# TaceoLabs/co-snarks

Measured on NVIDIA H100. Metric: co-Groth16 proofs/sec (BN254, 2^20 constraints); MSM Mscalar/s, higher is better.
Workload: dtype u32x8 (256-bit Montgomery, integer)

## Files before the change

### co_snarks_b200/csrc/cs_api.cu

```cuda
#include <stdarg.h>
#include "cs_lib.cuh"

namespace cs {

std::string& last_error() {
  static thread_local std::string e;
  return e;
}
int fail(int code, const char* fmt, ...) {
  char buf[1024];
  va_list ap;
  va_start(ap, fmt);
  vsnprintf(buf, sizeof(buf), fmt, ap);
  va_end(ap);
  last_error() = buf;
  return code;
}
#if !defined(CS_EMU)
__attribute__((constructor)) static void cs_more_hw_queues() { setenv("CUDA_DEVICE_MAX_CONNECTIONS", "32", 0); }
#endif

std::atomic<uint64_t>& launch_counter() {
  static std::atomic<uint64_t> c{0};
  return c;
}

int ctx_fork(cs_ctx* ctx, int nside) {
  if (ctx->msm_ws[0].profile) {
    if (!ctx->ev_t0) CS_CUDA(cudaEventCreateWithFlags(&ctx->ev_t0, 0));
    CS_CUDA(cudaEventRecord(ctx->ev_t0, ctx->stream));
  }
  CS_CUDA(cudaEventRecord(ctx->ev_fork, ctx->stream));
  for (int i = 0; i < nside; i++) CS_CUDA(cudaStreamWaitEvent(ctx->side[i], ctx->ev_fork, 0));
  return 0;
}
int ctx_join(cs_ctx* ctx, int nside) {
  for (int i = 0; i < nside; i++) {
    CS_CUDA(cudaEventRecord(ctx->ev_side[i], ctx->side[i]));
    CS_CUDA(cudaStreamWaitEvent(ctx->stream, ctx->ev_side[i], 0));
  }
  return 0;
}

template <class FrP>
static int ntt_smem_optin() {
#if !defined(CS_EMU)
#define CS_NTT_ATTR(D, S, KB) \
  CS_CUDA(cudaFuncSetAttribute(k_ntt_pass<FrP, D, S>, cudaFuncAttributeMaxDynamicSharedMemorySize, KB * 1024))
  CS_NTT_ATTR(true, false, 64); CS_NTT_ATTR(false, false, 64); CS_NTT_ATTR(true, true, 96); CS_NTT_ATTR(false, true, 96);
#undef CS_NTT_ATTR
#endif
  return 0;
}

}

using namespace cs;

extern "C" {

const char* cs_last_error(void) { return last_error().c_str(); }

const char* cs_version(void) {
#if defined(CS_EMU)
  return "cosnarks-b200 0.1 (CPU emulation build -- tests only)";
#else
  return "cosnarks-b200 0.1 (sm_90a)";
#endif
}

int cs_ctx_create(int device, void* stream, cs_ctx** out) {
  if (!out) return fail(CS_ERR_ARG, "cs_ctx_create: out is NULL");
  int ndev = 0;
  cudaError_t e = cudaGetDeviceCount(&ndev);
  if (e != cudaSuccess || ndev == 0)
    return fail(CS_ERR_CUDA, "cs_ctx_create: no CUDA device available (%s); this library has no CPU path",
                e != cudaSuccess ? cudaGetErrorString(e) : "device count 0");
  if (device < 0 || device >= ndev) return fail(CS_ERR_ARG, "cs_ctx_create: device %d out of range (%d devices)", device, ndev);
  CS_CUDA(cudaSetDevice(device));
  cs_ctx* ctx = new cs_ctx();
  ctx->device = device;
  int prio_side = -2, prio_acc = 0, prio_wm = -2;
  if (const char* e = getenv("CS_PRIO")) sscanf(e, "%d,%d,%d", &prio_side, &prio_acc, &prio_wm);
  const char* split_env = getenv("CS_MSM_SPLIT");
  const bool split = !(split_env && atoi(split_env) == 0);
  if (stream) {
    ctx->stream = (cudaStream_t)stream;
  } else {
    CS_CUDA(cudaStreamCreateWithPriority(&ctx->stream, cudaStreamNonBlocking, prio_side));
    ctx->own_stream = true;
  }
  for (int i = 0; i < CS_NSIDE; i++) {
    CS_CUDA(cudaStreamCreateWithPriority(&ctx->side[i], cudaStreamNonBlocking, prio_side));
    if (split) CS_CUDA(cudaStreamCreateWithPriority(&ctx->acc[i], cudaStreamNonBlocking, prio_acc));
    CS_CUDA(cudaEventCreateWithFlags(&ctx->ev_side[i], cudaEventDisableTiming));
  }
  CS_CUDA(cudaStreamCreateWithPriority(&ctx->wm, cudaStreamNonBlocking, prio_wm));
  CS_CUDA(cudaEventCreateWithFlags(&ctx->ev_wm, cudaEventDisableTiming));
  CS_CUDA(cudaEventCreateWithFlags(&ctx->ev_fork, cudaEventDisableTiming));
  CS_TRY(ntt_smem_optin<Bn254Fr>());
#if defined(CS_ENABLE_BLS12_381)
  CS_TRY(ntt_smem_optin<Bls381Fr>());
#endif
  *out = ctx;
  return 0;
}

void cs_ctx_destroy(cs_ctx* ctx) {
  if (!ctx) return;
  cudaSetDevice(ctx->device);
  cudaDeviceSynchronize();
  ctx->msm_ws[CS_WIT_SORT].release();
  for (int i = 0; i < CS_NSIDE; i++) {
    ctx->msm_ws[i].release();
    if (ctx->side[i]) cudaStreamDestroy(ctx->side[i]);
    if (ctx->acc[i]) cudaStreamDestroy(ctx->acc[i]);
    if (ctx->ev_side[i]) cudaEventDestroy(ctx->ev_side[i]);
  }
  if (ctx->ev_fork) cudaEventDestroy(ctx->ev_fork);
  if (ctx->wm) cudaStreamDestroy(ctx->wm);
  if (ctx->ev_wm) cudaEventDestroy(ctx->ev_wm);
  if (ctx->ev_t0) cudaEventDestroy(ctx->ev_t0);
  ctx->io.release();
  ctx->prf_keys.release();
  ctx->sc_part.release();
  ctx->sc_res.release();
  if (ctx->own_stream && ctx->stream) cudaStreamDestroy(ctx->stream);
  delete ctx;
}

int cs_ctx_synchronize(cs_ctx* ctx) {
  if (!ctx) return fail(CS_ERR_ARG, "ctx is NULL");
  CS_CUDA(cudaStreamSynchronize(ctx->stream));
  return 0;
}

uint64_t cs_ctx_launch_count(const cs_ctx*) { return launch_counter().load(); }

int cs_dev_alloc(cs_ctx* ctx, size_t bytes, void** d_out) {
  if (!ctx || !d_out) return fail(CS_ERR_ARG, "cs_dev_alloc: bad argument");
  CS_CUDA(cudaSetDevice(ctx->device));
  CS_CUDA(cudaMalloc(d_out, bytes ? bytes : 1));
  return 0;
}
int cs_dev_free(cs_ctx* ctx, void* d_ptr) {
  if (!ctx) return fail(CS_ERR_ARG, "ctx is NULL");
  CS_CUDA(cudaFree(d_ptr));
  return 0;
}
int cs_host_alloc_pinned(size_t bytes, void** h_out) {
  if (!h_out) return fail(CS_ERR_ARG, "h_out is NULL");
  CS_CUDA(cudaMallocHost(h_out, bytes ? bytes : 1));
  return 0;
}
int cs_host_free_pinned(void* h_ptr) {
  CS_CUDA(cudaFreeHost(h_ptr));
  return 0;
}
int cs_memcpy_h2d(cs_ctx* ctx, void* d_dst, const void* h_src, size_t bytes) {
  if (!ctx) return fail(CS_ERR_ARG, "ctx is NULL");
  CS_CUDA(cudaMemcpyAsync(d_dst, h_src, bytes, cudaMemcpyHostToDevice, ctx->stream));
  CS_CUDA(cudaStreamSynchronize(ctx->stream));
  return 0;
}
int cs_memcpy_d2h(cs_ctx* ctx, void* h_dst, const void* d_src, size_t bytes) {
  if (!ctx) return fail(CS_ERR_ARG, "ctx is NULL");
  CS_CUDA(cudaMemcpyAsync(h_dst, d_src, bytes, cudaMemcpyDeviceToHost, ctx->stream));
  CS_CUDA(cudaStreamSynchronize(ctx->stream));
  return 0;
}

}

namespace cs {

constexpr unsigned MSM_MAX_WINDOW = 20;
static_assert((1u << (MSM_MAX_WINDOW - 1)) + 1 <= MSM_SCAN_MAX_BLOCKS * MSM_SCAN_T, "MSM_MAX_WINDOW exceeds the scan");

template <class Cfg, int G>
int bases_upload_t(cs_ctx* ctx, const uint64_t* h_points, size_t n, int window_bits, cs_bases* b) {
  typedef typename GroupOf<Cfg, G>::F F;
  unsigned c = window_bits ? (unsigned)window_bits : msm_auto_window(n, Cfg::FR_BITS);
  if (c < 2 || c > MSM_MAX_WINDOW)
    return fail(CS_ERR_ARG, "cs_bases_upload: window_bits %d out of range [2,%u] (0 = automatic)", window_bits, MSM_MAX_WINDOW);
  b->sh = msm_shape(Cfg::FR_BITS, c);
  b->n = n;
  size_t total = (size_t)b->sh.W * n;
  if (total >= (1ull << 31)) return fail(CS_ERR_LIMIT, "cs_bases_upload: W*n = %zu exceeds 2^31", total);
  CS_TRY(b->table.reserve(total * sizeof(Affine<F>)));
  CS_CUDA(cudaMemcpyAsync(b->table.p, h_points, n * sizeof(Affine<F>), cudaMemcpyHostToDevice, ctx->stream));
  CS_TRY(b->infmask.reserve(((n + 31) / 32) * 4));
  CS_LAUNCH(k_msm_infmask<F>, ceil_div((n + 31) / 32, 128), 128, 0, ctx->stream, b->table.as<Affine<F>>(), (uint32_t)n,
            b->infmask.as<uint32_t>());
  CS_LAUNCH(k_msm_precompute<F>, ceil_div(n, 128), 128, 0, ctx->stream, b->table.as<Affine<F>>(), (uint32_t)n,
            b->sh.c, b->sh.W);
  if (G == 0 && std::is_same<Cfg, Bn254Cfg>::value) {
    static int f52_env = -1;
    if (f52_env < 0) { const char* e = getenv("CS_MSM_F52"); f52_env = e ? atoi(e) : 0; }
    if (f52_env) {
      const size_t ncoords = total * 2;
      CS_LAUNCH(k_msm_table_to_m260<Bn254Fq52 COMMA Bn254Fq>, ceil_div(ncoords, 128), 128, 0, ctx->stream,
                b->table.as<uint32_t>(), ncoords);
      b->m260 = true;
    }
  }
  CS_CUDA(cudaGetLastError());
  CS_CUDA(cudaStreamSynchronize(ctx->stream));
  return 0;
}

template <class Cfg, int G>
int msm_enqueue_t(cs_ctx* ctx, int slot, cudaStream_t st, const cs_bases* b, size_t offset,
                  const uint32_t* d_scalars, unsigned sstride, size_t n, int mont, int sort_slot, bool view) {
  typedef typename GroupOf<Cfg, G>::F F;
  return msm_enqueue<F, typename Cfg::FrP>(ctx->msm_ws[slot], b->table.as<Affine<F>>(), b->infmask.as<uint32_t>(), (uint32_t)b->n, b->sh,
                                           (uint32_t)offset, d_scalars, sstride, (uint32_t)n, mont, st,
                                           sort_slot >= 0 ? &ctx->msm_ws[sort_slot] : nullptr, view, b->m260, ctx->acc[slot]);
}

template <class Cfg, int G>
void msm_finish_t(cs_ctx* ctx, int slot, uint64_t* out_affine, int* out_inf) {
  typedef typename GroupOf<Cfg, G>::HF HF;
  const host::HXyzz<HF>* r = reinterpret_cast<const host::HXyzz<HF>*>(ctx->msm_ws[slot].h_result);
  host::HAffine<HF> a = host::haffine(*r);
  memcpy(out_affine, &a, sizeof(a));
  if (out_inf) *out_inf = a.is_inf() ? 1 : 0;
}

int msm_enqueue_dyn(cs_ctx* ctx, int slot, cudaStream_t st, const cs_bases* b, size_t offset,
                    const uint32_t* d_scalars, unsigned sstride, size_t n, int mont, int sort_slot, bool view) {
  CS_DISPATCH_CURVE(b->curve, {
    if (b->group == CS_G1) return msm_enqueue_t<Cfg, 0>(ctx, slot, st, b, offset, d_scalars, sstride, n, mont, sort_slot, view);
    return msm_enqueue_t<Cfg, 1>(ctx, slot, st, b, offset, d_scalars, sstride, n, mont, sort_slot, view);
  });
  return 0;
}
int msm_sort_shared_dyn(cs_ctx* ctx, int slot, cudaStream_t st, const cs_bases* b, const uint32_t* d_scalars,
                        unsigned sstride, size_t n, int mont) {
  CS_DISPATCH_CURVE(b->curve, {
    return msm_sort<typename Cfg::FrP>(ctx->msm_ws[slot], nullptr, (uint32_t)n, b->sh, 0, d_scalars, sstride, (uint32_t)n,
                                       mont, st);
  });
  return 0;
}

int msm_finish_dyn(cs_ctx* ctx, int slot, const cs_bases* b, uint64_t* out_affine, int* out_inf) {
  CS_DISPATCH_CURVE(b->curve, {
    if (b->group == CS_G1) msm_finish_t<Cfg, 0>(ctx, slot, out_affine, out_inf);
    else msm_finish_t<Cfg, 1>(ctx, slot, out_affine, out_inf);
  });
  return 0;
}

}

// ... 834 lines not shown
```

### co_snarks_b200/csrc/cs_msm.cuh

```cuda
#pragma once
#include <stdlib.h>
#include "cs_common.cuh"
#include "cs_curve.cuh"

namespace cs {

constexpr unsigned MSM_SLICE_MAX = 64;
constexpr unsigned MSM_ORDER_BLOCK = 256;
constexpr unsigned MSM_RED_SEG = 4;
constexpr unsigned MSM_SIGN = 0x80000000u;

template <class FrP>
CS_GLOBAL void k_msm_digits(const uint32_t* __restrict__ scalars, uint32_t sstride, uint32_t n, int mont,
                            uint32_t c, uint32_t W, const uint32_t* __restrict__ infmask, uint32_t offset,
                            uint32_t* __restrict__ dig, uint32_t* __restrict__ count) {
  uint32_t i = blockIdx.x * blockDim.x + threadIdx.x;
  if (i >= n) return;
  if (infmask && ((infmask[(offset + i) >> 5] >> ((offset + i) & 31)) & 1)) {
    for (uint32_t w = 0; w < W; w++) dig[(size_t)w * n + i] = 0;
    return;
  }
  Fp<FrP> s;
  const uint4* src = reinterpret_cast<const uint4*>(scalars) + (size_t)i * sstride * (FrP::N / 4);
  CS_UNROLL
  for (int k = 0; k < FrP::N / 4; k++) {
    uint4 v = src[k];
    s.l[4 * k] = v.x; s.l[4 * k + 1] = v.y; s.l[4 * k + 2] = v.z; s.l[4 * k + 3] = v.w;
  }
  if (mont) s = s.from_mont();
  uint32_t lim[FrP::N + 1];
  CS_UNROLL
  for (int k = 0; k < FrP::N; k++) lim[k] = s.l[k];
  lim[FrP::N] = 0;
  const uint32_t half = 1u << (c - 1);
  const uint32_t mask = (1u << c) - 1;
  uint32_t carry = 0;
  for (uint32_t w = 0; w < W; w++) {
    uint32_t pos = w * c;
    uint32_t li = pos >> 5, sh = pos & 31;
    uint32_t lo = li < FrP::N ? lim[li] : 0;
    uint32_t hi = li + 1 < FrP::N ? lim[li + 1] : 0;
    uint32_t d = (__funnelshift_r(lo, hi, sh) & mask) + carry;
    uint32_t out;
    if (d > half) {
      out = ((1u << c) - d) | MSM_SIGN;
      carry = 1;
    } else {
      out = d;
      carry = 0;
    }
    dig[(size_t)w * n + i] = out;
    uint32_t b = out & ~MSM_SIGN;
    if (b) atomicAdd(&count[b], 1u);
  }
}

template <class F>
CS_GLOBAL void k_msm_infmask(const Affine<F>* __restrict__ table, uint32_t n, uint32_t* __restrict__ mask) {
  uint32_t wd = blockIdx.x * blockDim.x + threadIdx.x;
  if (wd * 32 >= n) return;
  uint32_t m = 0;
  for (uint32_t k = 0; k < 32 && wd * 32 + k < n; k++)
    if (table[wd * 32 + k].is_inf()) m |= 1u << k;
  mask[wd] = m;
}

constexpr unsigned MSM_SCAN_T = 1024;
constexpr unsigned MSM_SCAN_MAX_BLOCKS = 1024;
CS_D void msm_scan_terms(const uint32_t* __restrict__ count, uint32_t k, uint32_t nb1, uint32_t S, uint32_t* v) {
  uint32_t cnt = (k && k < nb1) ? count[k] : 0;
  uint32_t n0 = (cnt + S - 1) / S;
  uint32_t n1 = (n0 + S - 1) / S;
  v[0] = cnt; v[1] = n0; v[2] = n1; v[3] = (n1 + S - 1) / S;
}
static CS_GLOBAL void k_msm_scan1(const uint32_t* __restrict__ count, uint32_t nb1 , uint32_t S,
                                  uint32_t* __restrict__ start, uint32_t* __restrict__ sstart0,
                                  uint32_t* __restrict__ sstart1, uint32_t* __restrict__ sstart2, uint32_t* __restrict__ aux) {
  __shared__ uint32_t sm[4][32];
  const uint32_t t = threadIdx.x, lane = t & 31, wid = t >> 5, nwarp = blockDim.x >> 5;
  const uint32_t k = blockIdx.x * blockDim.x + t;
  uint32_t v[4], inc[4];
  msm_scan_terms(count, k, nb1, S, v);
  CS_UNROLL
  for (int q = 0; q < 4; q++) {
    uint32_t x = v[q];
    CS_UNROLL
    for (uint32_t d = 1; d < 32; d <<= 1) {
      uint32_t y = __shfl_up_sync(0xffffffffu, x, d);
      if (lane >= d) x += y;
    }
    inc[q] = x;
    if (lane == 31) sm[q][wid] = x;
  }
  __syncthreads();
  uint32_t w[4], x[4];
  CS_UNROLL
  for (int q = 0; q < 4; q++) {
    w[q] = (wid == 0 && lane < nwarp) ? sm[q][lane] : 0;
    x[q] = w[q];
    CS_UNROLL
    for (uint32_t d = 1; d < 32; d <<= 1) {
      uint32_t y = __shfl_up_sync(0xffffffffu, x[q], d);
      if (lane >= d) x[q] += y;
    }
  }
  __syncthreads();
  if (wid == 0 && lane < nwarp) {
    CS_UNROLL
    for (int q = 0; q < 4; q++) sm[q][lane] = x[q] - w[q];
    if (lane == nwarp - 1) {
      CS_UNROLL
      for (int q = 0; q < 4; q++) aux[blockIdx.x * 4 + q] = x[q];
    }
  }
  __syncthreads();
  if (k < nb1) {
    start[k] = sm[0][wid] + inc[0] - v[0];
    sstart0[k] = sm[1][wid] + inc[1] - v[1];
    sstart1[k] = sm[2][wid] + inc[2] - v[2];
    sstart2[k] = sm[3][wid] + inc[3] - v[3];
  }
}
static CS_GLOBAL void k_msm_scan2(const uint32_t* __restrict__ count, uint32_t nb1, uint32_t S,
                                  uint32_t* __restrict__ start, uint32_t* __restrict__ sstart0,
                                  uint32_t* __restrict__ sstart1, uint32_t* __restrict__ sstart2,
                                  const uint32_t* __restrict__ aux) {
  const uint32_t k = blockIdx.x * blockDim.x + threadIdx.x;
  if (k >= nb1) return;
  uint32_t off[4] = {0, 0, 0, 0};
  for (uint32_t b = 0; b < blockIdx.x; b++) {
    CS_UNROLL
    for (int q = 0; q < 4; q++) off[q] += aux[b * 4 + q];
  }
  uint32_t a = start[k] + off[0], b0 = sstart0[k] + off[1], b1 = sstart1[k] + off[2], b2 = sstart2[k] + off[3];
  start[k] = a; sstart0[k] = b0; sstart1[k] = b1; sstart2[k] = b2;
  if (k == nb1 - 1) {
    uint32_t v[4];
    msm_scan_terms(count, k, nb1, S, v);
    start[nb1] = a + v[0]; sstart0[nb1] = b0 + v[1]; sstart1[nb1] = b1 + v[2]; sstart2[nb1] = b2 + v[3];
  }
}

static CS_GLOBAL void k_msm_scatter(const uint32_t* __restrict__ dig, uint32_t n, uint32_t nbases,
                             uint32_t offset, const uint32_t* __restrict__ start,
                             uint32_t* __restrict__ cursor, uint32_t* __restrict__ sorted) {
  uint32_t i = blockIdx.x * blockDim.x + threadIdx.x;
  uint32_t w = blockIdx.y;
  if (i >= n) return;
  uint32_t d = dig[(size_t)w * n + i];
  uint32_t b = d & ~MSM_SIGN;
  if (!b) return;
  uint32_t pos = start[b] + atomicAdd(&cursor[b], 1u);
  sorted[pos] = (w * nbases + offset + i) | (d & MSM_SIGN);
}

constexpr unsigned MSM_VIEW_T = 256;
constexpr unsigned MSM_VIEW_WORDS = MSM_VIEW_T / 32;

CS_D uint32_t popc32(uint32_t x) {
#if defined(CS_EMU)
  return (uint32_t)__builtin_popcount(x);
#else
  return __popc(x);
#endif
}
CS_D uint32_t warp_bits(bool pred) {
#if defined(CS_EMU)
  uint32_t x = pred ? 1u << (threadIdx.x & 31) : 0u;
  for (uint32_t d = 16; d > 0; d >>= 1) x += __shfl_xor_sync(0xffffffffu, x, d);
  return x;
#else
  return __ballot_sync(0xffffffffu, pred);
#endif
}

static CS_GLOBAL void k_msm_view_flags(const uint32_t* __restrict__ sorted, const uint32_t* __restrict__ src_start,
                                       uint32_t nb1, uint32_t n, const uint32_t* __restrict__ infmask, uint32_t offset,
                                       uint32_t* __restrict__ keep, uint32_t* __restrict__ blk_cnt) {
  __shared__ uint32_t cnt[MSM_VIEW_WORDS];
  const uint32_t t = threadIdx.x;
  const uint32_t p = blockIdx.x * MSM_VIEW_T + t;
  bool k = false;
  if (p < src_start[nb1]) {
    const uint32_t i = (sorted[p] & ~MSM_SIGN) % n;
    k = !((infmask[(offset + i) >> 5] >> ((offset + i) & 31)) & 1);
  }
  const uint32_t bits = warp_bits(k);
  if ((t & 31) == 0) {
    keep[(size_t)blockIdx.x * MSM_VIEW_WORDS + (t >> 5)] = bits;
    cnt[t >> 5] = popc32(bits);
  }
  __syncthreads();
  if (t == 0) {
    uint32_t c = 0;
    for (uint32_t w = 0; w < MSM_VIEW_WORDS; w++) c += cnt[w];
    blk_cnt[blockIdx.x] = c;
  }
}

static CS_GLOBAL void k_msm_view_scan(const uint32_t* __restrict__ blk_cnt, uint32_t nblk, uint32_t* __restrict__ blk_off) {
  __shared__ uint32_t sm[MSM_SCAN_T];
  const uint32_t t = threadIdx.x, T = blockDim.x;
  const uint32_t per = (nblk + T - 1) / T;
  const uint32_t lo = t * per < nblk ? t * per : nblk, hi = lo + per < nblk ? lo + per : nblk;
  uint32_t s = 0;
  for (uint32_t b = lo; b < hi; b++) s += blk_cnt[b];
  sm[t] = s;
  __syncthreads();
  for (uint32_t d = 1; d < T; d <<= 1) {
    const uint32_t v = t >= d ? sm[t - d] : 0;
    __syncthreads();
    sm[t] += v;
    __syncthreads();
  }
  uint32_t run = sm[t] - s;
  for (uint32_t b = lo; b < hi; b++) {
    const uint32_t c = blk_cnt[b];
    blk_off[b] = run;
    run += c;
  }
  if (t == T - 1) blk_off[nblk] = run;
}

CS_D uint32_t view_kept_before(uint32_t p, const uint32_t* __restrict__ keep, const uint32_t* __restrict__ blk_off) {
  const uint32_t blk = p / MSM_VIEW_T;
  uint32_t r = blk_off[blk];
  for (uint32_t w = blk * MSM_VIEW_WORDS; w < (p >> 5); w++) r += popc32(keep[w]);
  if (p & 31) r += popc32(keep[p >> 5] & ((1u << (p & 31)) - 1));
  return r;
}

static CS_GLOBAL void k_msm_view_counts(const uint32_t* __restrict__ src_start, uint32_t nb1, const uint32_t* __restrict__ keep,
                                        const uint32_t* __restrict__ blk_off, uint32_t* __restrict__ count) {
  const uint32_t b = blockIdx.x * blockDim.x + threadIdx.x;
  if (b >= nb1) return;
  count[b] = b ? view_kept_before(src_start[b + 1], keep, blk_off) - view_kept_before(src_start[b], keep, blk_off) : 0;
}

static CS_GLOBAL void k_msm_view_scatter(const uint32_t* __restrict__ sorted, uint32_t n, uint32_t nbases, uint32_t offset,
                                         const uint32_t* __restrict__ keep, const uint32_t* __restrict__ blk_off,
                                         uint32_t* __restrict__ out) {
  const uint32_t t = threadIdx.x;
  const uint32_t* kb = keep + (size_t)blockIdx.x * MSM_VIEW_WORDS;
  const uint32_t word = kb[t >> 5];
  if (!((word >> (t & 31)) & 1)) return;
  uint32_t pos = blk_off[blockIdx.x] + popc32(word & ((1u << (t & 31)) - 1));
  for (uint32_t k = 0; k < (t >> 5); k++) pos += popc32(kb[k]);
  const uint32_t e = sorted[blockIdx.x * MSM_VIEW_T + t];
  const uint32_t v = e & ~MSM_SIGN, w = v / n, i = v - w * n;
  out[pos] = (w * nbases + offset + i) | (e & MSM_SIGN);
}

CS_D uint32_t find_bucket(const uint32_t* __restrict__ arr, uint32_t nb1, uint32_t s) {
  uint32_t lo = 0, hi = nb1;
  while (hi - lo > 1) {
    uint32_t mid = (lo + hi) >> 1;
    if (arr[mid] <= s) lo = mid; else hi = mid;
  }
  return lo;
}

static CS_GLOBAL void k_msm_slice_hist(const uint32_t* __restrict__ count, const uint32_t* __restrict__ sstart0,
                                       uint32_t nb1, uint32_t S, uint32_t* __restrict__ slice_len,
                                       uint32_t* __restrict__ slice_bkt, uint32_t* __restrict__ block_hist) {
  __shared__ uint32_t h[MSM_SLICE_MAX + 1];
  for (uint32_t k = threadIdx.x; k <= MSM_SLICE_MAX; k += blockDim.x) h[k] = 0;
  __syncthreads();
  uint32_t s = blockIdx.x * blockDim.x + threadIdx.x;
  if (s < sstart0[nb1]) {
    uint32_t lo = 0, hi = nb1;
    while (hi - lo > 1) {
      uint32_t mid = (lo + hi) >> 1;
      if (sstart0[mid] <= s) lo = mid; else hi = mid;
    }
    uint32_t j = s - sstart0[lo];
    uint32_t len = count[lo] - j * S;
    if (len > S) len = S;
    slice_len[s] = len;
    slice_bkt[s] = lo;
    atomicAdd(&h[len], 1u);
  }
  __syncthreads();
  for (uint32_t k = threadIdx.x; k <= MSM_SLICE_MAX; k += blockDim.x)
    block_hist[(size_t)blockIdx.x * (MSM_SLICE_MAX + 1) + k] = h[k];
}

constexpr unsigned MSM_OFF_CHUNKS = 64;
static CS_GLOBAL void k_msm_slice_off1(const uint32_t* __restrict__ block_hist, uint32_t nblocks,
                                       uint32_t* __restrict__ chunk_sum) {
  uint32_t id = blockIdx.x * blockDim.x + threadIdx.x;
  if (id >= (MSM_SLICE_MAX + 1) * MSM_OFF_CHUNKS) return;
  uint32_t L = id / MSM_OFF_CHUNKS, ch = id % MSM_OFF_CHUNKS;
  uint32_t per = (nblocks + MSM_OFF_CHUNKS - 1) / MSM_OFF_CHUNKS;
  uint32_t lo = ch * per, hi = lo + per < nblocks ? lo + per : nblocks;
  uint32_t sum = 0;
  for (uint32_t b = lo; b < hi; b++) sum += block_hist[(size_t)b * (MSM_SLICE_MAX + 1) + L];
  chunk_sum[id] = sum;
}
static CS_GLOBAL void k_msm_slice_off2(uint32_t* __restrict__ chunk_sum, uint32_t* __restrict__ len_base) {
  uint32_t L = blockIdx.x * blockDim.x + threadIdx.x;
  if (L > MSM_SLICE_MAX) return;
  uint32_t run = 0;
  for (uint32_t c = 0; c < MSM_OFF_CHUNKS; c++) {
    uint32_t v = chunk_sum[L * MSM_OFF_CHUNKS + c];
    chunk_sum[L * MSM_OFF_CHUNKS + c] = run;
    run += v;
// ... 165 lines not shown
  Affine<F> p = table[i];
  if (p.is_inf()) {
    for (uint32_t w = 1; w < W; w++) table[(size_t)w * n + i] = Affine<F>::inf();
    return;
  }
  Xyzz<F> cur = Xyzz<F>::from_affine(p);
  uint32_t w = 1;
  while (w < W) {
    Xyzz<F> pts[MSM_PRE_CHUNK];
    F pre[MSM_PRE_CHUNK];
    int cnt = 0;
    bool degenerate = false;
    for (; cnt < MSM_PRE_CHUNK && w + cnt < W; cnt++) {
      for (uint32_t k = 0; k < c; k++) cur = dbl_xyzz(cur);
      pts[cnt] = cur;
      degenerate = degenerate || cur.is_inf();
    }
    Affine<F> last;
    if (degenerate) {
      for (int j = 0; j < cnt; j++) {
        last = to_affine(pts[j]);
        table[(size_t)(w + j) * n + i] = last;
      }
    } else {
      pre[0] = pts[0].zzz;
      for (int j = 1; j < cnt; j++) pre[j] = pre[j - 1] * pts[j].zzz;
      F inv = pre[cnt - 1].inverse();
      for (int j = cnt - 1; j >= 0; j--) {
        F zi = j ? inv * pre[j - 1] : inv;
        inv = inv * pts[j].zzz;
        F zzi = (zi * pts[j].zz).sqr();
        Affine<F> a;
        a.x = pts[j].x * zzi;
        a.y = pts[j].y * zi;
        table[(size_t)(w + j) * n + i] = a;
        if (j == cnt - 1) last = a;
      }
    }
    cur = Xyzz<F>::from_affine(last);
    w += cnt;
  }
}

template <class F, class FrP>
CS_GLOBAL void __launch_bounds__(128) k_fixed_base_mul(const Affine<F>* __restrict__ base,
                                                       const uint32_t* __restrict__ scalars, uint32_t n,
                                                       int mont, Affine<F>* __restrict__ out) {
  uint32_t i = blockIdx.x * blockDim.x + threadIdx.x;
  if (i >= n) return;
  Fp<FrP> s;
  const uint4* src = reinterpret_cast<const uint4*>(scalars) + (size_t)i * (FrP::N / 4);
  CS_UNROLL
  for (int k = 0; k < FrP::N / 4; k++) {
    uint4 v = src[k];
    s.l[4 * k] = v.x; s.l[4 * k + 1] = v.y; s.l[4 * k + 2] = v.z; s.l[4 * k + 3] = v.w;
  }
  if (mont) s = s.from_mont();
  uint32_t lim[FrP::N];
  CS_UNROLL
  for (int k = 0; k < FrP::N; k++) lim[k] = s.l[k];
  Affine<F> b = base[0];
  Xyzz<F> acc = Xyzz<F>::inf();
  for (int bit = FrP::N * 32 - 1; bit >= 0; bit--) {
    acc = dbl_xyzz(acc);
    if ((lim[bit >> 5] >> (bit & 31)) & 1) madd(acc, b, false);
  }
  out[i] = to_affine(acc);
}

struct MsmShape {
  uint32_t c, W, B;
};

static inline MsmShape msm_shape(uint32_t scalar_bits, uint32_t c) {
  MsmShape s;
  s.c = c;
  s.W = (scalar_bits + 1 + c - 1) / c;
  s.B = 1u << (c - 1);
  return s;
}

static inline uint32_t msm_auto_window(size_t n, uint32_t scalar_bits) {
  int lg = 0;
  while ((1ull << (lg + 1)) <= n) lg++;
  int c = lg >= 15 ? 16 : lg - 4;
  if (c < 4) c = 4;
  while (c < 16) {
    const uint32_t W = (scalar_bits + 1 + c - 1) / c;
    const uint32_t top = scalar_bits + 1 - (W - 1) * c;
    if (2 * top >= (uint32_t)c) break;
    c++;
  }
  return (uint32_t)c;
}
static inline uint32_t msm_slice(const MsmShape& sh) {
  const char* e = getenv("CS_MSM_SLICE");
  if (e && atoi(e) == 64) return 64u;
  if (e && atoi(e) == 32) return 32u;
  return sh.c >= 18 ? 64u : 32u;
}

constexpr int MSM_NSTAGE = 5;
struct MsmWorkspace {
  DevBuf dig, sorted, meta, part0, part1, part2, bucket, red, scal, result, order;
  void* h_result = nullptr;
  size_t h_result_cap = 0;
  bool profile = false;
  cudaEvent_t ev[MSM_NSTAGE + 1] = {};
  cudaEvent_t sorted_ev = nullptr;
  bool sorted_ev_made = false, sorted_once = false;
  cudaEvent_t acc_in = nullptr, acc_out = nullptr;
  int mark(int i, cudaStream_t st) {
    if (!profile) return 0;
    if (!ev[i]) CS_CUDA(cudaEventCreateWithFlags(&ev[i], 0));
    CS_CUDA(cudaEventRecord(ev[i], st));
    return 0;
  }
  void release() {
    for (int i = 0; i <= MSM_NSTAGE; i++) {
      if (ev[i]) cudaEventDestroy(ev[i]);
      ev[i] = nullptr;
    }
    if (sorted_ev_made) cudaEventDestroy(sorted_ev);
    if (acc_in) cudaEventDestroy(acc_in);
    if (acc_out) cudaEventDestroy(acc_out);
    acc_in = acc_out = nullptr;
    sorted_ev = nullptr;
    sorted_ev_made = sorted_once = false;
    dig.release(); sorted.release(); meta.release(); part0.release(); part1.release(); part2.release();
    bucket.release(); red.release(); scal.release(); result.release(); order.release();
    if (h_result) cudaFreeHost(h_result);
    h_result = nullptr;
    h_result_cap = 0;
  }
};

template <class F>
int msm_accum0_f52(const Affine<F>* table, const uint32_t* sorted, const uint32_t* count, const uint32_t* start,
                   const uint32_t* sstart0, uint32_t nb1, uint32_t S, const uint32_t* order, const uint32_t* order_b,
                   Xyzz<F>* part0, uint32_t max_s0, cudaStream_t st);

struct MsmSizes {
  uint32_t nb1, S, ob;
  size_t nent, max_s0, max_s1, max_s2;
  MsmSizes(const MsmShape& sh, uint32_t n) {
    nb1 = sh.B + 1;
    nent = (size_t)sh.W * n;
    S = msm_slice(sh);
    max_s0 = nent / S + nb1;
    max_s1 = max_s0 / S + nb1;
    max_s2 = max_s1 / S + nb1;
    ob = ceil_div(max_s0, MSM_ORDER_BLOCK);
  }
  size_t meta_words() const { return 2 * (size_t)nb1 + 4 * ((size_t)nb1 + 1) + 4 * MSM_SCAN_MAX_BLOCKS; }
  size_t order_words() const {
    return 4 * max_s0 + (size_t)ob * (MSM_SLICE_MAX + 1) + 2 * (MSM_SLICE_MAX + 1) + (size_t)(MSM_SLICE_MAX + 1) * MSM_OFF_CHUNKS;
  }
};
struct MsmSortBufs {
  uint32_t *count, *cursor, *start, *sstart0, *sstart1, *sstart2, *aux;
  uint32_t *slice_len, *slice_bkt, *order, *order_b, *block_hist, *len_base, *chunk_sum;
  MsmSortBufs(const MsmWorkspace& w, const MsmSizes& z) {
    count = w.meta.as<uint32_t>();
    cursor = count + z.nb1;
    start = cursor + z.nb1;
    sstart0 = start + z.nb1 + 1;
    sstart1 = sstart0 + z.nb1 + 1;
    sstart2 = sstart1 + z.nb1 + 1;
    aux = sstart2 + z.nb1 + 1;
    slice_len = w.order.as<uint32_t>();
    slice_bkt = slice_len + z.max_s0;
    order = slice_bkt + z.max_s0;
    order_b = order + z.max_s0;
    block_hist = order_b + z.max_s0;
    len_base = block_hist + (size_t)z.ob * (MSM_SLICE_MAX + 1);
    chunk_sum = len_base + 2 * (MSM_SLICE_MAX + 1);
  }
};

static inline int msm_check_limits(const MsmShape& sh, uint32_t n, uint32_t nbases) {
  const size_t nent = (size_t)sh.W * n;
  if (nent >= (1ull << 31) || (size_t)sh.W * nbases >= (1ull << 31))
    return fail(-3, "msm: W*n = %zu exceeds 2^31 entries", nent);
  return 0;
}

static inline int msm_scan(const MsmSortBufs& q, const MsmSizes& z, uint32_t B, cudaStream_t st) {
  const uint32_t sb = ceil_div(z.nb1, MSM_SCAN_T);
  if (sb > MSM_SCAN_MAX_BLOCKS) return fail(-3, "msm: %u buckets exceed the scan's limit", B);
  CS_LAUNCH_SYNC(k_msm_scan1, sb, MSM_SCAN_T, 0, st, q.count, z.nb1, z.S, q.start, q.sstart0, q.sstart1, q.sstart2, q.aux);
  CS_LAUNCH(k_msm_scan2, sb, MSM_SCAN_T, 0, st, q.count, z.nb1, z.S, q.start, q.sstart0, q.sstart1, q.sstart2, q.aux);
  return 0;
}

static inline int msm_slice_order(MsmWorkspace& ws, const MsmSortBufs& q, const MsmSizes& z, cudaStream_t st) {
  CS_LAUNCH_SYNC(k_msm_slice_hist, z.ob, MSM_ORDER_BLOCK, 0, st, q.count, q.sstart0, z.nb1, z.S, q.slice_len, q.slice_bkt,
                 q.block_hist);
  const uint32_t nt = (MSM_SLICE_MAX + 1) * MSM_OFF_CHUNKS;
  CS_LAUNCH(k_msm_slice_off1, ceil_div(nt, 128), 128, 0, st, q.block_hist, z.ob, q.chunk_sum);
  CS_LAUNCH(k_msm_slice_off2, 1, 128, 0, st, q.chunk_sum, q.len_base);
  CS_LAUNCH(k_msm_slice_off3, ceil_div(nt, 128), 128, 0, st, q.block_hist, z.ob, q.chunk_sum, q.len_base);
  CS_LAUNCH_SYNC(k_msm_slice_order, z.ob, MSM_ORDER_BLOCK, 0, st, q.slice_len, q.slice_bkt, (uint32_t)z.max_s0, q.sstart0,
                 z.nb1, q.block_hist, q.len_base, q.order, q.order_b);
  if (!ws.sorted_ev_made) {
    CS_CUDA(cudaEventCreateWithFlags(&ws.sorted_ev, cudaEventDisableTiming));
    ws.sorted_ev_made = true;
  }
  CS_CUDA(cudaEventRecord(ws.sorted_ev, st));
  ws.sorted_once = true;
  return 0;
}

template <class FrP>
int msm_sort(MsmWorkspace& ws, const uint32_t* infmask, uint32_t nbases, MsmShape sh, uint32_t offset,
             const uint32_t* d_scalars, uint32_t sstride, uint32_t n, int mont, cudaStream_t st) {
  CS_TRY(msm_check_limits(sh, n, nbases));
  const MsmSizes z(sh, n);
  CS_TRY(ws.dig.reserve(z.nent * 4));
  CS_TRY(ws.sorted.reserve(z.nent * 4));
  CS_TRY(ws.meta.reserve(z.meta_words() * 4));
  CS_TRY(ws.order.reserve(z.order_words() * 4));
  const MsmSortBufs q(ws, z);
  CS_TRY(ws.mark(0, st));
  CS_CUDA(cudaMemsetAsync(q.count, 0, 2 * (size_t)z.nb1 * 4, st));
  CS_LAUNCH(k_msm_digits<FrP>, ceil_div(n, 256), 256, 0, st, d_scalars, sstride, n, mont, sh.c, sh.W, infmask, offset,
            ws.dig.as<uint32_t>(), q.count);
  CS_TRY(ws.mark(1, st));
  CS_TRY(msm_scan(q, z, sh.B, st));
  CS_LAUNCH(k_msm_scatter, dim3(ceil_div(n, 256), sh.W), 256, 0, st, ws.dig.as<uint32_t>(), n, nbases, offset, q.start,
            q.cursor, ws.sorted.as<uint32_t>());
  return msm_slice_order(ws, q, z, st);
}

static inline int msm_view(MsmWorkspace& ws, const MsmWorkspace& src, const uint32_t* infmask, uint32_t nbases,
                           MsmShape sh, uint32_t offset, uint32_t n, cudaStream_t st) {
  const MsmSizes z(sh, n);
  const uint32_t nblk = ceil_div(z.nent, MSM_VIEW_T);
  CS_TRY(ws.dig.reserve(((size_t)nblk * MSM_VIEW_WORDS + 2 * (size_t)nblk + 1) * 4));
  CS_TRY(ws.sorted.reserve(z.nent * 4));
  CS_TRY(ws.meta.reserve(z.meta_words() * 4));
  CS_TRY(ws.order.reserve(z.order_words() * 4));
  const MsmSortBufs q(ws, z), s(src, z);
  uint32_t* keep = ws.dig.as<uint32_t>();
  uint32_t* blk_cnt = keep + (size_t)nblk * MSM_VIEW_WORDS;
  uint32_t* blk_off = blk_cnt + nblk;
  const uint32_t* src_sorted = src.sorted.as<uint32_t>();
  CS_LAUNCH_SYNC(k_msm_view_flags, nblk, MSM_VIEW_T, 0, st, src_sorted, s.start, z.nb1, n, infmask, offset, keep, blk_cnt);
  CS_LAUNCH_SYNC(k_msm_view_scan, 1, MSM_SCAN_T, 0, st, blk_cnt, nblk, blk_off);
  CS_LAUNCH(k_msm_view_counts, ceil_div(z.nb1, 256), 256, 0, st, s.start, z.nb1, keep, blk_off, q.count);
  CS_LAUNCH(k_msm_view_scatter, nblk, MSM_VIEW_T, 0, st, src_sorted, n, nbases, offset, keep, blk_off,
            ws.sorted.as<uint32_t>());
  CS_TRY(msm_scan(q, z, sh.B, st));
  return msm_slice_order(ws, q, z, st);
}

template <class F, class FrP>
int msm_enqueue(MsmWorkspace& ws, const Affine<F>* table, const uint32_t* infmask, uint32_t nbases, MsmShape sh,
                uint32_t offset,
                const uint32_t* d_scalars, uint32_t sstride, uint32_t n, int mont, cudaStream_t st,
                MsmWorkspace* sort_from = nullptr, bool view = false, bool table_m260 = false, cudaStream_t st_acc = nullptr) {
  CS_TRY(msm_check_limits(sh, n, nbases));
  const MsmSizes z(sh, n);
  const uint32_t nb1 = z.nb1, S = z.S;
  const size_t max_s0 = z.max_s0, max_s1 = z.max_s1, max_s2 = z.max_s2;
  CS_TRY(ws.part0.reserve(max_s0 * sizeof(Xyzz<F>)));
  CS_TRY(ws.part1.reserve(max_s1 * sizeof(Xyzz<F>)));
  CS_TRY(ws.part2.reserve(max_s2 * sizeof(Xyzz<F>)));
  CS_TRY(ws.bucket.reserve((size_t)nb1 * sizeof(Xyzz<F>)));
  const uint32_t L = sh.B < MSM_RED_SEG ? sh.B : MSM_RED_SEG;
  const uint32_t nseg = (sh.B + L - 1) / L;
  const uint32_t fs_threads = sizeof(Xyzz<F>) > 128 ? 128 : 256;
  const uint32_t fs_blocks = nseg > 4 * fs_threads ? (nseg + fs_threads - 1) / fs_threads : 1;
  CS_TRY(ws.red.reserve(((size_t)nseg + fs_blocks) * sizeof(Xyzz<F>)));
  CS_TRY(ws.result.reserve(sizeof(Xyzz<F>)));
  if (ws.h_result_cap < sizeof(Xyzz<F>)) {
    if (ws.h_result) cudaFreeHost(ws.h_result);
    CS_CUDA(cudaMallocHost(&ws.h_result, sizeof(Xyzz<F>)));
    ws.h_result_cap = sizeof(Xyzz<F>);
  }
  if (sort_from) {
    if (!sort_from->sorted_once) return fail(-1, "msm: the workspace to share a sort with has not been enqueued");
    CS_TRY(ws.mark(0, st));
    CS_CUDA(cudaStreamWaitEvent(st, sort_from->sorted_ev, 0));
    CS_TRY(ws.mark(1, st));
    if (view) CS_TRY(msm_view(ws, *sort_from, infmask, nbases, sh, offset, n, st));
  } else {
    CS_TRY(msm_sort<FrP>(ws, infmask, nbases, sh, offset, d_scalars, sstride, n, mont, st));
  }
  MsmWorkspace& so = sort_from && !view ? *sort_from : ws;
  const MsmSortBufs q(so, z);
  const uint32_t *count = q.count, *start = q.start, *sstart0 = q.sstart0, *sstart1 = q.sstart1, *sstart2 = q.sstart2;
  const uint32_t *order = q.order, *order_b = q.order_b;
  CS_TRY(ws.mark(2, st));
  cudaStream_t st_main = st;
  if (st_acc) {
    if (!ws.acc_in) {
      CS_CUDA(cudaEventCreateWithFlags(&ws.acc_in, cudaEventDisableTiming));
      CS_CUDA(cudaEventCreateWithFlags(&ws.acc_out, cudaEventDisableTiming));
    }
    CS_CUDA(cudaEventRecord(ws.acc_in, st));
    CS_CUDA(cudaStreamWaitEvent(st_acc, ws.acc_in, 0));
    st = st_acc;
  }
  {
    static int minb_env = -1;
    if (minb_env < 0) { const char* e = getenv("CS_ACCUM0_MINB"); minb_env = e ? atoi(e) : 0; }
    const int minb = minb_env ? minb_env : (sizeof(Affine<F>) > 64 ? 2 : 4);
    if (table_m260) {
      CS_TRY((msm_accum0_f52<F>(table, so.sorted.as<uint32_t>(), count, start, sstart0, nb1, S, order, order_b,
                                ws.part0.as<Xyzz<F>>(), (uint32_t)max_s0, st)));
    } else {
#define CS_ACC0(M)                                                                                              \
  CS_LAUNCH(k_msm_accum0<F COMMA M>, ceil_div(max_s0, 128), 128, 0, st, table, so.sorted.as<uint32_t>(), count, \
            start, sstart0, nb1, S, order, order_b, ws.part0.as<Xyzz<F>>())
    switch (minb) {
      case 2: CS_ACC0(2); break;
      case 3: CS_ACC0(3); break;
      case 5: CS_ACC0(5); break;
      case 6: CS_ACC0(6); break;
      default: CS_ACC0(4); break;
    }
#undef CS_ACC0
    }
  }
  if (st_acc) {
    CS_CUDA(cudaEventRecord(ws.acc_out, st_acc));
    st = st_main;
    CS_CUDA(cudaStreamWaitEvent(st, ws.acc_out, 0));
  }
  CS_TRY(ws.mark(3, st));
  CS_LAUNCH(k_msm_accum1<F>, ceil_div(max_s1, 128), 128, 0, st, ws.part0.as<Xyzz<F>>(), sstart0, sstart1,
            nb1, S, ws.part1.as<Xyzz<F>>());
  CS_LAUNCH(k_msm_accum1<F>, ceil_div(max_s2, 128), 128, 0, st, ws.part1.as<Xyzz<F>>(), sstart1, sstart2,
            nb1, S, ws.part2.as<Xyzz<F>>());
  CS_LAUNCH(k_msm_accum2<F>, ceil_div(nb1, 128), 128, 0, st, ws.part2.as<Xyzz<F>>(), sstart2, nb1,
            ws.bucket.as<Xyzz<F>>());
  CS_TRY(ws.mark(4, st));
  CS_LAUNCH(k_msm_reduce_seg<F>, ceil_div(nseg, 128), 128, 0, st, ws.bucket.as<Xyzz<F>>(), sh.B, L,
            ws.red.as<Xyzz<F>>());
  if (fs_blocks > 1) {
    Xyzz<F>* stage = ws.red.as<Xyzz<F>>() + nseg;
    CS_LAUNCH_SYNC(k_msm_final_sum<F>, fs_blocks, fs_threads, fs_threads * sizeof(Xyzz<F>), st, ws.red.as<Xyzz<F>>(), nseg,
                   stage);
    CS_LAUNCH_SYNC(k_msm_final_sum<F>, 1, fs_threads, fs_threads * sizeof(Xyzz<F>), st, stage, fs_blocks,
                   ws.result.as<Xyzz<F>>());
  } else {
    CS_LAUNCH_SYNC(k_msm_final_sum<F>, 1, fs_threads, fs_threads * sizeof(Xyzz<F>), st, ws.red.as<Xyzz<F>>(), nseg,
                   ws.result.as<Xyzz<F>>());
  }
  CS_TRY(ws.mark(5, st));
  CS_CUDA(cudaMemcpyAsync(ws.h_result, ws.result.p, sizeof(Xyzz<F>), cudaMemcpyDeviceToHost, st));
  CS_CUDA(cudaGetLastError());
  return 0;
}

}
```

Baseline: 49.76.

## Replace global-atomic MSM bucket sort with tiled shared-memory histogram and scatter

Result: faster. 51.44 (median of 6 runs) (+3.4%).

```diff
diff --git a/co_snarks_b200/csrc/cs_api.cu b/co_snarks_b200/csrc/cs_api.cu
--- a/co_snarks_b200/csrc/cs_api.cu
+++ b/co_snarks_b200/csrc/cs_api.cu
@@ -99,8 +99,10 @@
   CS_CUDA(cudaEventCreateWithFlags(&ctx->ev_wm, cudaEventDisableTiming));
   CS_CUDA(cudaEventCreateWithFlags(&ctx->ev_fork, cudaEventDisableTiming));
   CS_TRY(ntt_smem_optin<Bn254Fr>());
+  CS_TRY(msm_smem_optin<Bn254Fr>());
 #if defined(CS_ENABLE_BLS12_381)
   CS_TRY(ntt_smem_optin<Bls381Fr>());
+  CS_TRY(msm_smem_optin<Bls381Fr>());
 #endif
   *out = ctx;
   return 0;
diff --git a/co_snarks_b200/csrc/cs_msm.cuh b/co_snarks_b200/csrc/cs_msm.cuh
--- a/co_snarks_b200/csrc/cs_msm.cuh
+++ b/co_snarks_b200/csrc/cs_msm.cuh
@@ -10,16 +10,9 @@
 constexpr unsigned MSM_RED_SEG = 4;
 constexpr unsigned MSM_SIGN = 0x80000000u;
 
-template <class FrP>
-CS_GLOBAL void k_msm_digits(const uint32_t* __restrict__ scalars, uint32_t sstride, uint32_t n, int mont,
-                            uint32_t c, uint32_t W, const uint32_t* __restrict__ infmask, uint32_t offset,
-                            uint32_t* __restrict__ dig, uint32_t* __restrict__ count) {
-  uint32_t i = blockIdx.x * blockDim.x + threadIdx.x;
-  if (i >= n) return;
-  if (infmask && ((infmask[(offset + i) >> 5] >> ((offset + i) & 31)) & 1)) {
-    for (uint32_t w = 0; w < W; w++) dig[(size_t)w * n + i] = 0;
-    return;
-  }
+template <class FrP, class Fn>
+CS_D void msm_recode(const uint32_t* __restrict__ scalars, uint32_t sstride, uint32_t i, int mont, uint32_t c,
+                     uint32_t W, Fn&& f) {
   Fp<FrP> s;
   const uint4* src = reinterpret_cast<const uint4*>(scalars) + (size_t)i * sstride * (FrP::N / 4);
   CS_UNROLL
@@ -28,18 +21,14 @@
     s.l[4 * k] = v.x; s.l[4 * k + 1] = v.y; s.l[4 * k + 2] = v.z; s.l[4 * k + 3] = v.w;
   }
   if (mont) s = s.from_mont();
-  uint32_t lim[FrP::N + 1];
-  CS_UNROLL
-  for (int k = 0; k < FrP::N; k++) lim[k] = s.l[k];
-  lim[FrP::N] = 0;
   const uint32_t half = 1u << (c - 1);
   const uint32_t mask = (1u << c) - 1;
   uint32_t carry = 0;
   for (uint32_t w = 0; w < W; w++) {
     uint32_t pos = w * c;
     uint32_t li = pos >> 5, sh = pos & 31;
-    uint32_t lo = li < FrP::N ? lim[li] : 0;
-    uint32_t hi = li + 1 < FrP::N ? lim[li + 1] : 0;
+    uint32_t lo = li < FrP::N ? s.l[li] : 0;
+    uint32_t hi = li + 1 < FrP::N ? s.l[li + 1] : 0;
     uint32_t d = (__funnelshift_r(lo, hi, sh) & mask) + carry;
     uint32_t out;
     if (d > half) {
@@ -49,9 +38,88 @@
       out = d;
       carry = 0;
     }
-    dig[(size_t)w * n + i] = out;
-    uint32_t b = out & ~MSM_SIGN;
-    if (b) atomicAdd(&count[b], 1u);
+    f(w, out);
+  }
+}
+
+CS_D bool msm_base_inf(const uint32_t* __restrict__ infmask, uint32_t k) {
+  return infmask && ((infmask[k >> 5] >> (k & 31)) & 1);
+}
+
+constexpr unsigned MSM_BIN_T = 1024;
+constexpr unsigned MSM_BIN_TILE = 4096;
+constexpr unsigned MSM_BIN_SPAN = 1u << 15;
+constexpr unsigned MSM_SCATTER_SPAN = 1u << 13;
+
+template <class FrP>
+CS_GLOBAL void __launch_bounds__(MSM_BIN_T) k_msm_bin_count(const uint32_t* __restrict__ scalars, uint32_t sstride,
+                                                            uint32_t n, int mont, uint32_t c, uint32_t W,
+                                                            const uint32_t* __restrict__ infmask, uint32_t offset,
+                                                            uint32_t tile, uint32_t B, uint32_t* __restrict__ tab) {
+  CS_DYN_SMEM(uint32_t, h);
+  const uint32_t lo = blockIdx.y * MSM_BIN_SPAN + 1;
+  const uint32_t span = B + 1 - lo < MSM_BIN_SPAN ? B + 1 - lo : MSM_BIN_SPAN;
+  for (uint32_t k = threadIdx.x; k < span; k += blockDim.x) h[k] = 0;
+  __syncthreads();
+  const uint32_t i1 = (blockIdx.x + 1) * tile < n ? (blockIdx.x + 1) * tile : n;
+  for (uint32_t i = blockIdx.x * tile + threadIdx.x; i < i1; i += blockDim.x) {
+    if (msm_base_inf(infmask, offset + i)) continue;
+    msm_recode<FrP>(scalars, sstride, i, mont, c, W, [&](uint32_t, uint32_t d) {
+      const uint32_t k = (d & ~MSM_SIGN) - lo;
+      if (k < span) atomicAdd(&h[k], 1u);
+    });
+  }
+  __syncthreads();
+  uint32_t* row = tab + (size_t)blockIdx.x * B + (lo - 1);
+  for (uint32_t k = threadIdx.x; k < span; k += blockDim.x) row[k] = h[k];
+}
+
+constexpr unsigned MSM_BIN_SCAN_U = 16;
+static CS_GLOBAL void k_msm_bin_scan(uint32_t* __restrict__ tab, uint32_t nblk, uint32_t B, uint32_t* __restrict__ count) {
+  const uint32_t b = blockIdx.x * blockDim.x + threadIdx.x;
+  if (b == 0) count[0] = 0;
+  if (b >= B) return;
+  uint32_t* col = tab + b;
+  uint32_t run = 0, r = 0;
+  for (; r + MSM_BIN_SCAN_U <= nblk; r += MSM_BIN_SCAN_U) {
+    uint32_t v[MSM_BIN_SCAN_U];
+    CS_UNROLL
+    for (uint32_t u = 0; u < MSM_BIN_SCAN_U; u++) v[u] = col[(size_t)(r + u) * B];
+    CS_UNROLL
+    for (uint32_t u = 0; u < MSM_BIN_SCAN_U; u++) {
+      col[(size_t)(r + u) * B] = run;
+      run += v[u];
+    }
+  }
+  for (; r < nblk; r++) {
+    const uint32_t v = col[(size_t)r * B];
+    col[(size_t)r * B] = run;
+    run += v;
+  }
+  count[b + 1] = run;
+}
+
+template <class FrP>
+CS_GLOBAL void __launch_bounds__(MSM_BIN_T) k_msm_bin_scatter(const uint32_t* __restrict__ scalars, uint32_t sstride,
+                                                              uint32_t n, int mont, uint32_t c, uint32_t W,
+                                                              const uint32_t* __restrict__ infmask, uint32_t offset,
+                                                              uint32_t tile, uint32_t B, uint32_t nbases,
+                                                              const uint32_t* __restrict__ tab,
+                                                              const uint32_t* __restrict__ start,
+                                                              uint32_t* __restrict__ sorted) {
+  CS_DYN_SMEM(uint32_t, cur);
+  const uint32_t lo = blockIdx.y * MSM_SCATTER_SPAN + 1;
+  const uint32_t span = B + 1 - lo < MSM_SCATTER_SPAN ? B + 1 - lo : MSM_SCATTER_SPAN;
+  const uint32_t* row = tab + (size_t)blockIdx.x * B + (lo - 1);
+  for (uint32_t k = threadIdx.x; k < span; k += blockDim.x) cur[k] = start[lo + k] + row[k];
+  __syncthreads();
+  const uint32_t i1 = (blockIdx.x + 1) * tile < n ? (blockIdx.x + 1) * tile : n;
+  for (uint32_t i = blockIdx.x * tile + threadIdx.x; i < i1; i += blockDim.x) {
+    if (msm_base_inf(infmask, offset + i)) continue;
+    msm_recode<FrP>(scalars, sstride, i, mont, c, W, [&](uint32_t w, uint32_t d) {
+      const uint32_t k = (d & ~MSM_SIGN) - lo;
+      if (k < span) sorted[atomicAdd(&cur[k], 1u)] = (w * nbases + offset + i) | (d & MSM_SIGN);
+    });
   }
 }
 
@@ -139,19 +207,6 @@
     msm_scan_terms(count, k, nb1, S, v);
     start[nb1] = a + v[0]; sstart0[nb1] = b0 + v[1]; sstart1[nb1] = b1 + v[2]; sstart2[nb1] = b2 + v[3];
   }
-}
-
-static CS_GLOBAL void k_msm_scatter(const uint32_t* __restrict__ dig, uint32_t n, uint32_t nbases,
-                             uint32_t offset, const uint32_t* __restrict__ start,
-                             uint32_t* __restrict__ cursor, uint32_t* __restrict__ sorted) {
-  uint32_t i = blockIdx.x * blockDim.x + threadIdx.x;
-  uint32_t w = blockIdx.y;
-  if (i >= n) return;
-  uint32_t d = dig[(size_t)w * n + i];
-  uint32_t b = d & ~MSM_SIGN;
-  if (!b) return;
-  uint32_t pos = start[b] + atomicAdd(&cursor[b], 1u);
-  sorted[pos] = (w * nbases + offset + i) | (d & MSM_SIGN);
 }
 
 constexpr unsigned MSM_VIEW_T = 256;
@@ -623,18 +678,17 @@
     max_s2 = max_s1 / S + nb1;
     ob = ceil_div(max_s0, MSM_ORDER_BLOCK);
   }
-  size_t meta_words() const { return 2 * (size_t)nb1 + 4 * ((size_t)nb1 + 1) + 4 * MSM_SCAN_MAX_BLOCKS; }
+  size_t meta_words() const { return (size_t)nb1 + 4 * ((size_t)nb1 + 1) + 4 * MSM_SCAN_MAX_BLOCKS; }
   size_t order_words() const {
     return 4 * max_s0 + (size_t)ob * (MSM_SLICE_MAX + 1) + 2 * (MSM_SLICE_MAX + 1) + (size_t)(MSM_SLICE_MAX + 1) * MSM_OFF_CHUNKS;
   }
 };
 struct MsmSortBufs {
-  uint32_t *count, *cursor, *start, *sstart0, *sstart1, *sstart2, *aux;
+  uint32_t *count, *start, *sstart0, *sstart1, *sstart2, *aux;
   uint32_t *slice_len, *slice_bkt, *order, *order_b, *block_hist, *len_base, *chunk_sum;
   MsmSortBufs(const MsmWorkspace& w, const MsmSizes& z) {
     count = w.meta.as<uint32_t>();
-    cursor = count + z.nb1;
-    start = cursor + z.nb1;
+    start = count + z.nb1;
     sstart0 = start + z.nb1 + 1;
     sstart1 = sstart0 + z.nb1 + 1;
     sstart2 = sstart1 + z.nb1 + 1;
@@ -683,23 +737,47 @@
 }
 
 template <class FrP>
+int msm_smem_optin() {
+#if !defined(CS_EMU)
+  CS_CUDA(cudaFuncSetAttribute(k_msm_bin_count<FrP>, cudaFuncAttributeMaxDynamicSharedMemorySize, MSM_BIN_SPAN * 4));
+  CS_CUDA(cudaFuncSetAttribute(k_msm_bin_scatter<FrP>, cudaFuncAttributeMaxDynamicSharedMemorySize, MSM_SCATTER_SPAN * 4));
+#endif
+  return 0;
+}
+
+static inline uint32_t msm_bin_tile(const MsmShape& sh, const MsmSizes& z, uint32_t n) {
+  const size_t rows = z.nent / sh.B > 1 ? z.nent / sh.B : 1;
+  const size_t nblk = ceil_div(n, MSM_BIN_TILE) < rows ? ceil_div(n, MSM_BIN_TILE) : rows;
+  return n ? ceil_div(n, nblk) : 1;
+}
+
+template <class FrP>
 int msm_sort(MsmWorkspace& ws, const uint32_t* infmask, uint32_t nbases, MsmShape sh, uint32_t offset,
              const uint32_t* d_scalars, uint32_t sstride, uint32_t n, int mont, cudaStream_t st) {
   CS_TRY(msm_check_limits(sh, n, nbases));
   const MsmSizes z(sh, n);
-  CS_TRY(ws.dig.reserve(z.nent * 4));
+  const uint32_t tile = msm_bin_tile(sh, z, n);
+  const uint32_t nblk = n ? ceil_div(n, tile) : 0;
+  const dim3 grid(nblk, ceil_div(sh.B, MSM_BIN_SPAN)), grid_sc(nblk, ceil_div(sh.B, MSM_SCATTER_SPAN));
+  const uint32_t smem = (sh.B < MSM_BIN_SPAN ? sh.B : MSM_BIN_SPAN) * 4;
+  const uint32_t smem_sc = (sh.B < MSM_SCATTER_SPAN ? sh.B : MSM_SCATTER_SPAN) * 4;
+  const size_t tab_words = (size_t)nblk * sh.B;
+  CS_TRY(ws.dig.reserve((tab_words > z.nent ? tab_words : z.nent) * 4));
   CS_TRY(ws.sorted.reserve(z.nent * 4));
   CS_TRY(ws.meta.reserve(z.meta_words() * 4));
   CS_TRY(ws.order.reserve(z.order_words() * 4));
   const MsmSortBufs q(ws, z);
+  uint32_t* tab = ws.dig.as<uint32_t>();
   CS_TRY(ws.mark(0, st));
-  CS_CUDA(cudaMemsetAsync(q.count, 0, 2 * (size_t)z.nb1 * 4, st));
-  CS_LAUNCH(k_msm_digits<FrP>, ceil_div(n, 256), 256, 0, st, d_scalars, sstride, n, mont, sh.c, sh.W, infmask, offset,
-            ws.dig.as<uint32_t>(), q.count);
+  if (nblk)
+    CS_LAUNCH_SYNC(k_msm_bin_count<FrP>, grid, MSM_BIN_T, smem, st, d_scalars, sstride, n, mont, sh.c, sh.W, infmask,
+                   offset, tile, sh.B, tab);
   CS_TRY(ws.mark(1, st));
+  CS_LAUNCH(k_msm_bin_scan, ceil_div(sh.B, 256), 256, 0, st, tab, nblk, sh.B, q.count);
   CS_TRY(msm_scan(q, z, sh.B, st));
-  CS_LAUNCH(k_msm_scatter, dim3(ceil_div(n, 256), sh.W), 256, 0, st, ws.dig.as<uint32_t>(), n, nbases, offset, q.start,
-            q.cursor, ws.sorted.as<uint32_t>());
+  if (nblk)
+    CS_LAUNCH_SYNC(k_msm_bin_scatter<FrP>, grid_sc, MSM_BIN_T, smem_sc, st, d_scalars, sstride, n, mont, sh.c, sh.W, infmask,
+                   offset, tile, sh.B, nbases, tab, q.start, ws.sorted.as<uint32_t>());
   return msm_slice_order(ws, q, z, st);
 }
 
```
